# liuzm-slam/VLOAM-NOTED

Measured on AMD Instinct MI355X. Metric: scan-to-map LM iters/sec on 64-ring KITTI-shaped cloud, higher is better.
Workload: dtype fp64 pose/normal equations, fp32 points

## Files before the change

### vloam-noted_amd/csrc/mapper.hip

```cpp
#include <algorithm>
#include <cmath>
#include <cstdlib>
#include <array>
#include <cstring>
#include <deque>
#include <vector>

#include "common.h"
#include "device_math.h"
#include "cellhash.h"
#include "comm.h"
#include "cubeindex.h"
#include "lm.h"
#include "voxel.h"
#include "voxel_hot.h"
#include "voxel_pcl.h"
#include "mapper_dev.h"
#include "mapper_stack.h"
#include "mapper_frame.h"
#include "mapper_corr.h"
#include "mapper_lm.h"
#include "mapper_map.h"

namespace loam {
// ... 191 lines not shown
  while (p < v) p <<= 1;
  return p;
}

void free_all(loam_mapper* h) {
  if (h->D.lm_peer && h->comm) {
    comm_peer_release(h->comm);
    h->D.lm_peer = nullptr;
    h->D.lm_peer_flag = nullptr;
  }
  for (void* p : h->ipc_open) (void)hipIpcCloseMemHandle(p);
  h->ipc_open.clear();
  if (h->ipc_own) (void)hipFree(h->ipc_own);
  h->ipc_own = nullptr;
  h->D.ipc_tab = nullptr;
  for (void* p : h->allocs) (void)hipFree(p);
  h->allocs.clear();
  if (h->d_pub) (void)hipFree(h->d_pub);
  h->d_pub = nullptr;
  h->pub_cap = 0;
  for (auto& gp : h->gexec)
    for (auto& g : gp)
      if (g) (void)hipGraphExecDestroy(g);
  for (auto& e : h->ev_pool) (void)hipEventDestroy(e);
  if (h->ev_stack) (void)hipEventDestroy(h->ev_stack);
  for (ParitySlot& S : h->slot)
    for (hipEvent_t e : {S.ev_sin, S.ev_fr[0], S.ev_fr[1]})
      if (e) (void)hipEventDestroy(e);
  h->ev_pool.clear();
  if (h->ev_opt_begin) (void)hipEventDestroy(h->ev_opt_begin);
  if (h->ev_opt_end) (void)hipEventDestroy(h->ev_opt_end);
  if (h->st) (void)hipStreamDestroy(h->st);
  if (h->st2) (void)hipStreamDestroy(h->st2);
}

void host_initial_guess(HostStream& H, double* pose) {
  dq qm{H.q_wmap_wodom[0], H.q_wmap_wodom[1], H.q_wmap_wodom[2], H.q_wmap_wodom[3]};
  dq qo{H.q_wodom[0], H.q_wodom[1], H.q_wodom[2], H.q_wodom[3]};
  dq q = qmul(qm, qo);
  d3 r = qrot(qm, d3{H.t_wodom[0], H.t_wodom[1], H.t_wodom[2]});
  pose[0] = q.x; pose[1] = q.y; pose[2] = q.z; pose[3] = q.w;
  pose[4] = r.x + H.t_wmap_wodom[0];
  pose[5] = r.y + H.t_wmap_wodom[1];
  pose[6] = r.z + H.t_wmap_wodom[2];
}

void host_transform_update(HostStream& H) {
  dq qw{H.pose[0], H.pose[1], H.pose[2], H.pose[3]};
  dq qo{H.q_wodom[0], H.q_wodom[1], H.q_wodom[2], H.q_wodom[3]};
  dq qm = qmul(qw, qinv(qo));
  d3 r = qrot(qm, d3{H.t_wodom[0], H.t_wodom[1], H.t_wodom[2]});
  H.q_wmap_wodom[0] = qm.x; H.q_wmap_wodom[1] = qm.y; H.q_wmap_wodom[2] = qm.z; H.q_wmap_wodom[3] = qm.w;
  H.t_wmap_wodom[0] = H.pose[4] - r.x;
  H.t_wmap_wodom[1] = H.pose[5] - r.y;
  H.t_wmap_wodom[2] = H.pose[6] - r.z;
}

StreamFrame fresh_record() {
  StreamFrame F{};
  F.cen[0] = 10; F.cen[1] = 10; F.cen[2] = 5;
  F.pose[3] = F.wodom[3] = F.wmap[3] = 1.0;
  return F;
}

void pack7(const double* q, const double* t, double* x) {
  std::copy(q, q + 4, x);
  std::copy(t, t + 3, x + 4);
}
void unpack7(const double* x, double* q, double* t) {
  std::copy(x, x + 4, q);
  std::copy(x + 4, x + 7, t);
}

int32_t check_stream(loam_mapper* h, int32_t s) {
  if (!h) {
    set_error("null mapper handle");
    return LOAM_ERR_ARG;
  }
  if (s < 0 || s >= h->B) {
    set_error("stream index out of range");
    return LOAM_ERR_ARG;
  }
  return LOAM_OK;
}

void bind_stack_parity(const loam_mapper* h, MapperDev& D, int par) {
  const ParitySlot& S = h->slot[par];
  D.sin = S.sin_buf;
  D.stk_n = S.stk_n_buf;
  D.stk_err = S.stk_err_buf;
  for (int m = 0; m < 2; ++m) D.stack[m] = S.stack_buf[m];
}

}

extern "C" {

static int32_t ipc_peer_setup(loam_mapper* h) {
  loam_comm* c = h->comm;
  MapperDev& D = h->D;
  const int R = c->size, me = c->rank;
  const size_t B = h->B, nslot = 2 * B * 2 * LM_MAX_PASSES * LM_NACC;
  const size_t bytes = nslot * sizeof(double) + B * 2 * sizeof(uint32_t);
  struct Msg {
    hipIpcMemHandle_t hdl;
    int32_t ok, pad;
  };
  static_assert(sizeof(Msg) % 8 == 0, "exchange record");
  Msg mine{};
  void* buf = nullptr;
  if (hipExtMallocWithFlags(&buf, bytes, hipDeviceMallocUncached) != hipSuccess) {
    (void)hipGetLastError();
    buf = nullptr;
    if (hipMalloc(&buf, bytes) != hipSuccess) {
      (void)hipGetLastError();
      buf = nullptr;
    }
  }
  mine.ok = buf && hipMemset(buf, 0, bytes) == hipSuccess && hipDeviceSynchronize() == hipSuccess &&
            hipIpcGetMemHandle(&mine.hdl, buf) == hipSuccess;
  if (!mine.ok) (void)hipGetLastError();
  Msg* dsend = nullptr;
  Msg* drecv = nullptr;
  std::vector<Msg> all(R);
  auto cleanup = [&] {
    if (dsend) (void)hipFree(dsend);
    if (drecv) (void)hipFree(drecv);
    dsend = drecv = nullptr;
  };
  LOAM_HIP(hipMalloc(&dsend, sizeof(Msg)));
  if (hipMalloc(&drecv, sizeof(Msg) * R) != hipSuccess) {
    cleanup();
    return LOAM_ERR_HIP;
  }
  auto exchange = [&]() -> int32_t {
    if (hipMemcpy(dsend, &mine, sizeof(Msg), hipMemcpyHostToDevice) != hipSuccess) return LOAM_ERR_HIP;
    TRY(comm_allgather(c, dsend, drecv, (int64_t)sizeof(Msg), h->st));
    if (hipStreamSynchronize(h->st) != hipSuccess ||
        hipMemcpy(all.data(), drecv, sizeof(Msg) * R, hipMemcpyDeviceToHost) != hipSuccess)
      return LOAM_ERR_HIP;
    return LOAM_OK;
  };
  int32_t rc = exchange();
  bool ok = rc == LOAM_OK;
  for (int r = 0; r < R && ok; ++r) ok = all[r].ok != 0;
  std::vector<unsigned long long> tab(2 * (size_t)R, 0ull);
  if (ok) {
    for (int r = 0; r < R; ++r) {
      void* p = buf;
      if (r != me) {
        p = nullptr;
        if (hipIpcOpenMemHandle(&p, all[r].hdl, hipIpcMemLazyEnablePeerAccess) != hipSuccess) {
          (void)hipGetLastError();
          p = nullptr;
        } else {
          h->ipc_open.push_back(p);
        }
      }
      tab[r] = reinterpret_cast<unsigned long long>(p);
      tab[R + r] = p ? reinterpret_cast<unsigned long long>(static_cast<char*>(p) + nslot * sizeof(double)) : 0ull;
      if (!p) ok = false;
    }
    const hipIpcMemHandle_t keep = mine.hdl;
    mine = Msg{};
    mine.hdl = keep;
    mine.ok = ok ? 1 : 0;
    if (rc == LOAM_OK) rc = exchange();
    ok = rc == LOAM_OK;
    for (int r = 0; r < R && ok; ++r) ok = all[r].ok != 0;
  }
  cleanup();
  if (!ok) {
    for (void* p : h->ipc_open) (void)hipIpcCloseMemHandle(p);
    h->ipc_open.clear();
    if (buf) (void)hipFree(buf);
    return rc;
  }
  h->ipc_own = buf;
  unsigned long long* dtab = nullptr;
  const int32_t arc = dalloc(h, &dtab, tab.size());
  if (arc != LOAM_OK) return arc;
  LOAM_HIP(hipMemcpyAsync(dtab, tab.data(), sizeof(unsigned long long) * tab.size(), hipMemcpyHostToDevice, h->st));
  LOAM_HIP(hipStreamSynchronize(h->st));
  D.ipc_tab = dtab;
  D.ipc_B = (int)B;
  return LOAM_OK;
}

static int32_t mapper_create(const loam_params* p, int32_t device, int32_t n_streams, loam_comm* comm,
                             loam_mapper** out) {
  if (!out || n_streams <= 0) {
    set_error("loam_mapper_create: bad arguments");
    return LOAM_ERR_ARG;
  }
  *out = nullptr;
  TRY(ensure_device(device));
  LOAM_HIP(hipSetDevice(device));
  vh_spin_limit_from_env(device);
  lm_peer_spin_limit_from_env(device);
  auto* h = new loam_mapper;
  if (p) h->P = *p; else loam_params_default(&h->P);
  h->dev = device;
  h->B = n_streams;
  h->comm = comm;
  MapperDev& D = h->D;
  D.B = n_streams;
  if (comm) {
    D.sharded = 1;
    D.rank = comm->rank;
    D.nrank = comm->size;
  }
  D.max_in = h->P.max_input_points;
  D.map_cap = h->P.max_map_points;
  D.sub_cap = h->P.max_submap_points;
  D.scratch_cap = D.sub_cap + D.max_in;
  {
    const uint64_t cap = (uint64_t)D.map_cap, margin = (uint64_t)D.sub_cap + 2ull * D.max_in;
    h->compact_at = (uint32_t)std::max<uint64_t>(cap / 2, cap > margin ? cap - margin : 0);
    D.compact_at = h->compact_at;
    D.compact_due_at = h->compact_at;
  }
  D.max_chunks = LM_EBLK;
  {
    int occ = 0, cus = 0;
    const char* env = std::getenv("LOAM_LM_PERSISTENT");
    const bool allow = !(env && env[0] == '0');
    if (hipDeviceGetAttribute(&cus, hipDeviceAttributeMultiprocessorCount, device) == hipSuccess && cus > 0)
      h->n_cu = cus;
    const bool peer = comm && comm->size > 1 && comm->kind == 2;
    const char* ienv = std::getenv("LOAM_PEER_LM");
    const bool ipc = comm && comm->size > 1 && comm->kind != 2 && !(ienv && ienv[0] == '0');
    h->want_ipc = false;
    if (allow && (!comm || comm->size == 1 || peer || ipc) &&
        hipOccupancyMaxActiveBlocksPerMultiprocessor(&occ, k_lm_round, LM_THREADS, 0) == hipSuccess &&
        hipDeviceGetAttribute(&cus, hipDeviceAttributeMultiprocessorCount, device) == hipSuccess) {
      occ = std::min(occ, 1);
      const int cap = occ * cus;
      h->lm_G = std::min(LM_EBLK, std::min(16, cap / (peer ? lm_padded(n_streams) * comm->size : n_streams)));
      const char* genv = std::getenv("LOAM_LM_G");
      if (genv && std::atoi(genv) > 0) h->lm_G = std::min(LM_EBLK, std::atoi(genv));
      if (ipc && h->lm_G > 0) {
        if (lm_padded(n_streams) * comm->size <= cap) h->want_ipc = true;
        else h->lm_G = 0;
      }
      if (peer && h->lm_G > 0) {
        const size_t nd = (size_t)2 * n_streams * 2 * comm->size * LM_MAX_PASSES * LM_NACC;
        void* pb = nullptr;
        if (comm_peer_buffer(comm, nd * sizeof(double) + (size_t)n_streams * 2 * comm->size * sizeof(uint32_t),
                             lm_padded(n_streams) * comm->size, cap, &pb) == LOAM_OK) {
          D.lm_peer = static_cast<double*>(pb);
          D.lm_peer_flag = reinterpret_cast<uint32_t*>(D.lm_peer + nd);
        } else {
          h->lm_G = 0;
        }
      }
    }
  }
  D.pcl_order = h->P.exact_voxel_order ? 1 : 0;
  D.stack_k = (n_streams <= 4 && !D.pcl_order) ? 8 : 0;
  if (const char* kenv = std::getenv("LOAM_STACK_K"))
    if (D.stack_k) D.stack_k = std::max(1, std::min(STACK_K_MAX, std::atoi(kenv)));
  D.leaf[0] = (float)h->P.mapping_line_resolution;
  D.leaf[1] = (float)h->P.mapping_plane_resolution;
  const size_t B = n_streams;
  auto fail = [&](int32_t rc) {
    free_all(h);
    delete h;
    return rc;
  };
  int32_t rc = LOAM_OK;
#define ALLOC(ptr, n) \
  if ((rc = dalloc(h, &(ptr), (n))) != LOAM_OK) return fail(rc)
  if (hipStreamCreateWithFlags(&h->st, hipStreamNonBlocking) != hipSuccess) return fail(LOAM_ERR_HIP);
  if (hipStreamCreateWithFlags(&h->st2, hipStreamNonBlocking) != hipSuccess) return fail(LOAM_ERR_HIP);
  if (hipEventCreate(&h->ev_opt_begin) != hipSuccess || hipEventCreate(&h->ev_opt_end) != hipSuccess ||
      hipEventCreateWithFlags(&h->ev_stack, hipEventDisableTiming) != hipSuccess)
    return fail(LOAM_ERR_HIP);
  for (ParitySlot& S : h->slot)
    if (hipEventCreateWithFlags(&S.ev_sin, hipEventDisableTiming) != hipSuccess ||
        hipEventCreate(&S.ev_fr[0]) != hipSuccess || hipEventCreate(&S.ev_fr[1]) != hipSuccess)
      return fail(LOAM_ERR_HIP);
  {
    const char* denv = std::getenv("LOAM_DEFER_EVERY");
    D.defer_every = denv ? std::max(0, std::atoi(denv)) : 0;
  }
  h->use_graph = n_streams <= 4 ? 1 : 0;
  h->knn_cs = n_streams <= 4 ? 8 : 0;
  D.knn_blk = n_streams <= 4 ? 4 * CORR_BLK : CORR_BLK;
  if (const char* benv = std::getenv("LOAM_KNN_BLK"))
    if (h->knn_cs) D.knn_blk = std::max(1, std::min(64 * CORR_BLK, std::atoi(benv)));
  ALLOC(D.fr, B);
  for (int m = 0; m < 2; ++m) {
    ALLOC(D.in_pts[m], B * D.max_in);
    for (ParitySlot& S : h->slot) ALLOC(S.stack_buf[m], B * D.max_in);
  }
  ALLOC(D.arena, B * 2 * 2 * (size_t)D.map_cap);
  ALLOC(D.carena, B * 2 * 2 * (size_t)D.map_cap);
  ALLOC(D.ctab, B * 2 * 2 * 4 * (size_t)D.map_cap);
  ALLOC(h->cube_tab[0], B * 2 * NCUBE);
  ALLOC(h->cube_tab[1], B * 2 * NCUBE);
  ALLOC(D.extra_flag, B * 2 * NCUBE);
  D.knn_stride = B * 2 * (size_t)D.max_in;
  ALLOC(D.knn_id, 5 * D.knn_stride);
  ALLOC(D.r_type, B * 2 * (size_t)D.max_in);
  ALLOC(D.r_px, B * 2 * (size_t)D.max_in);
  ALLOC(D.r_py, B * 2 * (size_t)D.max_in);
  ALLOC(D.r_pz, B * 2 * (size_t)D.max_in);
  for (int k = 0; k < 3; ++k) {
    ALLOC(D.r_a[k], B * 2 * (size_t)D.max_in);
    ALLOC(D.r_b[k], B * 2 * (size_t)D.max_in);
  }
  ALLOC(D.ins_pts, B * 2 * (size_t)D.max_in);
  ALLOC(D.ins_tag, B * 2 * (size_t)D.max_in);
  ALLOC(D.ins_sorted, B * 2 * (size_t)D.max_in);
  ALLOC(D.ins_off, B * 2 * (size_t)(INS_SLOTS + 1));
  ALLOC(D.stable_tok, B * 2 * (size_t)NCUBE);
  ALLOC(h->tok_tmp, B * 2 * (size_t)NCUBE);
  ALLOC(D.dbg, LOAM_DEBUG_COUNTERS);
  {
    const char* penv = std::getenv("LOAM_PHASE_COUNTERS");
    D.pdbg = (penv && std::atoi(penv) > 0) ? D.dbg : nullptr;
  }
  ALLOC(D.vx_pts, B * 2 * (size_t)D.scratch_cap);
  if (D.pcl_order) {
    const size_t ps = mp_scratch(D);
    ALLOC(D.pe, B * 2 * ps);
    ALLOC(D.pa, B * 2 * ps);
    ALLOC(D.pb, B * 2 * ps);
    ALLOC(D.ps, B * 2 * ps);
    ALLOC(D.pseg, B * 2 * (mp_pseg(ps) + 9));
  }
  ALLOC(D.vx_idx, B * 2 * (size_t)D.scratch_cap);
  ALLOC(D.stk_part, B * 2 * (size_t)STACK_K_MAX);
  for (ParitySlot& S : h->slot) {
    ALLOC(S.stk_n_buf, B * 2);
    ALLOC(S.stk_err_buf, B);
    if (B <= 4) {
      if (!(S.sin_buf = S.hsin.assign_mapped(B, StackIn{}))) return fail(LOAM_ERR_HIP);
    } else {
      ALLOC(S.sin_buf, B);
      if (!S.hsin.assign(B, StackIn{})) return fail(LOAM_ERR_HIP);
    }
  }
  bind_stack_parity(h, D, 0);
  ALLOC(h->d_stk_ready, 2);
  ALLOC(D.stk_pts, B * 2 * (size_t)D.max_in);
  ALLOC(D.stk_idx, B * 2 * (size_t)D.max_in);
  ALLOC(D.partials, B * (size_t)D.max_chunks * LM_NACC);
  ALLOC(D.lm_sync, B * 2 * LM_SYNC_WORDS);
  ALLOC(D.lm_xpub, B * 2 * 8);
  ALLOC(D.tickets, B);
  ALLOC(D.lm_tick, B);
  D.rq_cap = B * 2 * INS_SLOTS;
  ALLOC(D.rq, (size_t)RQ_CLASSES * D.rq_cap);
  ALLOC(D.rq_ctl, RQ_CLASSES);
  ALLOC(h->d_map_off, 2 * NCUBE + 1);
  ALLOC(h->d_new_off, B * 2 * (NCUBE + 1));
  if (D.sharded) {
    for (int m = 0; m < 2; ++m) D.blk_v[m] = shard_block_voxels(D.leaf[m]);
    const size_t nq = B * 2 * (size_t)D.max_in;
    NnRec* recv = nullptr;
    ALLOC(D.wcnt, B * 2 * (size_t)WIN_MAX);
    ALLOC(D.nn_send, nq);
    if (D.nrank > 1) {
      ALLOC(recv, nq * D.nrank);
      D.nn_recv = recv;
    } else {
      D.nn_recv = D.nn_send;
    }
    ALLOC(D.nn_xyz, 5 * nq);
    ALLOC(D.lm_red, B * (size_t)LM_NACC);
    ALLOC(D.pose_x, (size_t)D.nrank * B * 8);
    ALLOC(h->d_q_off, B + 1);
    D.q_off = h->d_q_off;
    if (!h->q_off.assign(2 * (B + 1), 0)) return fail(LOAM_ERR_HIP);
    if (D.nrank == 1) {
      for (size_t s = 0; s <= B; ++s) h->q_off[s] = (int)(s * 2 * (size_t)D.max_in);
      if (hipMemcpyAsync(h->d_q_off, h->q_off.data(), sizeof(int) * (B + 1), hipMemcpyHostToDevice, h->st) !=
          hipSuccess)
        return fail(LOAM_ERR_HIP);
    }
  }
#undef ALLOC
  D.cube_tab = h->cube_tab[0];
  if (!h->hf.assign(B, StreamFrame{})) return fail(LOAM_ERR_HIP);
  for (ParitySlot& S : h->slot)
    if (!(S.hfo_dev = S.hfo.assign_mapped(B, StreamFrame{})) || !(S.fin_dev = S.fin.assign_mapped(B, FrameIn{})) ||
        !(S.hfo_early_dev = S.hfo_early.assign_mapped(B, StreamFrame{})))
      return fail(LOAM_ERR_HIP);
  if (!(h->done_dev = h->done.assign_mapped(2, 0ull)) || !(h->done_early_dev = h->done_early.assign_mapped(2, 0ull)))
    return fail(LOAM_ERR_HIP);
  h->hs.assign(B, HostStream{});
  h->last_tail.assign(B, std::array<uint32_t, 2>{0u, 0u});
  for (size_t s = 0; s < B; ++s) h->hf[s] = fresh_record();
  if (hipStreamSynchronize(h->st) != hipSuccess) return fail(LOAM_ERR_HIP);
  if (h->want_ipc) {
    if ((rc = ipc_peer_setup(h)) != LOAM_OK) return fail(rc);
    if (!D.ipc_tab) h->lm_G = 0;
  }
  *out = h;
  return LOAM_OK;
}

int32_t loam_mapper_create(const loam_params* p, int32_t device, int32_t n_streams, loam_mapper** out) {
  return mapper_create(p, device, n_streams, nullptr, out);
}

int32_t loam_mapper_create_sharded(const loam_params* p, int32_t device, int32_t n_streams, loam_comm* comm,
                                   loam_mapper** out) {
  if (!comm) {
    set_error("loam_mapper_create_sharded: null comm");
    return LOAM_ERR_ARG;
  }
  return mapper_create(p, device, n_streams, comm, out);
}

int32_t loam_shard_owner(const float* xyz, float leaf, int32_t nrank) {
  if (!xyz || !(leaf > 0.f) || nrank < 1) return LOAM_ERR_ARG;
  return shard_owner(xyz[0], xyz[1], xyz[2], 1.0f / leaf, shard_block_voxels(leaf), nrank);
}

static int32_t finish_oldest(loam_mapper* h);
static int32_t settle_all(loam_mapper* h);
static bool chain_capable(const loam_mapper* h);
#define SETTLE(h)                                \
  do {                                           \
    if ((h) && !(h)->q.empty()) {                \
      LOAM_HIP(hipSetDevice((h)->dev));          \
      TRY(settle_all(h));                        \
    }                                            \
  } while (0)
#define SETTLE_RESULTS(h)                                                                   \
  do {                                                                                      \
    if ((h) && !(h)->q.empty() && !(h)->q.front().behind && !(h)->q.front().early_seen) { \
      LOAM_HIP(hipSetDevice((h)->dev));                                                     \
      TRY(finish_oldest(h));                                                                \
    }                                                                                       \
  } while (0)

int32_t loam_mapper_destroy(loam_mapper* h) {
  if (!h) return LOAM_ERR_ARG;
  (void)hipSetDevice(h->dev);
  while (!h->q.empty()) (void)finish_oldest(h);
  (void)hipStreamSynchronize(h->st);
  (void)hipStreamSynchronize(h->st2);
  free_all(h);
  delete h;
  return LOAM_OK;
}

int32_t loam_mapper_reset(loam_mapper* h) {
  if (!h) return LOAM_ERR_ARG;
  SETTLE(h);
  LOAM_HIP(hipSetDevice(h->dev));
  LOAM_HIP(hipStreamSynchronize(h->st2));
  for (int p = 0; p < 2; ++p)
    LOAM_HIP(hipMemsetAsync(h->cube_tab[p], 0, sizeof(uint2) * h->B * 2 * NCUBE, h->st));
  LOAM_HIP(hipMemsetAsync(h->D.stable_tok, 0, sizeof(uint32_t) * h->B * 2 * NCUBE, h->st));
  LOAM_HIP(hipStreamSynchronize(h->st));
  for (int s = 0; s < h->B; ++s) {
    h->hf[s] = fresh_record();
    h->last_tail[s] = {0u, 0u};
    h->hs[s] = HostStream{};
  }
  return LOAM_OK;
}

static int32_t mapper_input_common(loam_mapper* h, int32_t s, const float* corner, int32_t nc,
                                   const float* surf, int32_t ns, const double* q_wodom,
                                   const double* t_wodom, int32_t skip, hipMemcpyKind kind) {
  TRY(check_stream(h, s));
  if (!q_wodom || !t_wodom || nc < 0 || ns < 0 || (nc > 0 && !corner) || (ns > 0 && !surf)) {
    set_error("loam_mapper_input: bad arguments");
    return LOAM_ERR_ARG;
  }
  if (nc > h->D.max_in || ns > h->D.max_in) {
    set_error("loam_mapper_input: cloud larger than max_input_points");
    return LOAM_ERR_CAPACITY;
  }
  LOAM_HIP(hipSetDevice(h->dev));
  HostStream& H = h->hs[s];
  if (skip) {
    SETTLE(h);
    for (int i = 0; i < 4; ++i) H.q_wodom[i] = q_wodom[i];
    for (int i = 0; i < 3; ++i) H.t_wodom[i] = t_wodom[i];
    H.skip = true;
    double pose[7];
    host_initial_guess(H, pose);
    unpack7(pose, H.q_hf, H.t_hf);
    H.in_ready = false;
    H.stk_launched = false;
    return LOAM_OK;
  }
  if (kind == hipMemcpyHostToDevice) {
    H.in_p[0] = h->D.in_pts[0] + (size_t)s * h->D.max_in;
    H.in_p[1] = h->D.in_pts[1] + (size_t)s * h->D.max_in;
    if (nc) LOAM_HIP(hipMemcpyAsync((void*)H.in_p[0], corner, sizeof(float4) * nc, kind, h->st2));
    if (ns) LOAM_HIP(hipMemcpyAsync((void*)H.in_p[1], surf, sizeof(float4) * ns, kind, h->st2));
  } else {
    H.in_p[0] = reinterpret_cast<const float4*>(corner);
    H.in_p[1] = reinterpret_cast<const float4*>(surf);
  }
  H.in_n[0] = nc;
  H.in_n[1] = ns;
  for (int i = 0; i < 4; ++i) H.in_q[i] = q_wodom[i];
  for (int i = 0; i < 3; ++i) H.in_t[i] = t_wodom[i];
  H.skip = false;
  H.in_ready = true;
  H.stk_launched = false;
  return LOAM_OK;
}

int32_t loam_mapper_input(loam_mapper* h, int32_t s, const float* corner, int32_t nc, const float* surf,
                          int32_t ns, const double* q_wodom, const double* t_wodom, int32_t skip) {
  return mapper_input_common(h, s, corner, nc, surf, ns, q_wodom, t_wodom, skip, hipMemcpyHostToDevice);
}

int32_t loam_mapper_input_device(loam_mapper* h, int32_t s, const float* corner, int32_t nc,
                                 const float* surf, int32_t ns, const double* q_wodom,
                                 const double* t_wodom, int32_t skip) {
  return mapper_input_common(h, s, corner, nc, surf, ns, q_wodom, t_wodom, skip, hipMemcpyDeviceToDevice);
}

static hipError_t prof_begin(loam_mapper* h, int fam, hipEvent_t* stop, hipStream_t st) {
  *stop = nullptr;
  if (!h->prof) return hipSuccess;
  size_t k = h->ev_fam.size() * 2;
  while (h->ev_pool.size() < k + 2) {
    hipEvent_t e;
    hipError_t err = hipEventCreate(&e);
    if (err != hipSuccess) return err;
    h->ev_pool.push_back(e);
  }
  h->ev_fam.push_back(fam);
  *stop = h->ev_pool[k + 1];
  return hipEventRecord(h->ev_pool[k], st);
}
struct ProfStop {
  hipEvent_t ev = nullptr;
  hipStream_t st = nullptr;
  hipError_t end() {
    const hipError_t e = ev ? hipEventRecord(ev, st) : hipSuccess;
    ev = nullptr;
    return e;
  }
  ~ProfStop() { (void)end(); }
};
#define LAUNCH_ON(stream, fam, ...)                     \
  do {                                                  \
    ProfStop stop_;                                     \
    stop_.st = (stream);                                \
    LOAM_HIP(prof_begin(h, (fam), &stop_.ev, (stream))); \
    __VA_ARGS__;                                        \
    LOAM_HIP(stop_.end());                              \
  } while (0)
#define LAUNCH(fam, ...) LAUNCH_ON(h->st, fam, __VA_ARGS__)

int32_t loam_mapper_input_device_batch(loam_mapper* h, int32_t n, const int32_t* streams,
                                       const uint64_t* d_corner, const int32_t* n_corner,
                                       const uint64_t* d_surf, const int32_t* n_surf,
                                       const double* q_wodom, const double* t_wodom) {
  if (!h || n < 0 || (n > 0 && (!streams || !d_corner || !n_corner || !d_surf || !n_surf || !q_wodom || !t_wodom))) {
    set_error("loam_mapper_input_device_batch: bad arguments");
    return LOAM_ERR_ARG;
  }
  for (int i = 0; i < n; ++i) {
    int32_t rc = mapper_input_common(h, streams[i], reinterpret_cast<const float*>(d_corner[i]), n_corner[i],
                                     reinterpret_cast<const float*>(d_surf[i]), n_surf[i], q_wodom + 4 * i,
                                     t_wodom + 3 * i, 0, hipMemcpyDeviceToDevice);
    if (rc != LOAM_OK) return rc;
  }
  return LOAM_OK;
}

int32_t loam_mapper_lm_path(loam_mapper* h) {
  if (!h) return LOAM_ERR_ARG;
  if (h->lm_G <= 0) return 0;
  if (h->D.lm_peer) return 2;
  if (h->D.ipc_tab) return 3;
  return 1;
}

int64_t loam_mapper_total_iterations(loam_mapper* h) {
  if (!h) return LOAM_ERR_ARG;
  SETTLE_RESULTS(h);
  int64_t it = 0;
  for (int s = 0; s < h->B; ++s)
    if (h->hs[s].solved_last) it += h->hs[s].st.lm[0].iterations + h->hs[s].st.lm[1].iterations;
  return it;
}

int32_t loam_mapper_stats_all(loam_mapper* h, loam_map_stats* out, int32_t n) {
  SETTLE_RESULTS(h);
  if (!h || !out || n < 0 || n > h->B) return LOAM_ERR_ARG;
  for (int s = 0; s < n; ++s) out[s] = h->hs[s].st;
  return LOAM_OK;
}

static int32_t launch_stacks(loam_mapper* h) {
  const int par = h->spar, B = h->B;
  for (const FrameRec& R : h->q)
    if (R.fpar == par) return LOAM_OK;
  bool any = false;
  ParitySlot& S = h->slot[par];
  LOAM_HIP(hipEventSynchronize(S.ev_sin));
  StackIn* in = S.hsin.data();
// ... 820 lines not shown
```

### vloam-noted_amd/csrc/mapper_corr.h

```cpp
#pragma once

namespace loam {

struct Near5 {
  float d[5];
  int id[5];
  int pos[5];
};
__device__ inline void near5_offer(Near5& T, float d, int id, int pos) {
  if (!(d < T.d[4] || (d == T.d[4] && id < T.id[4]))) return;
  T.d[4] = d; T.id[4] = id; T.pos[4] = pos;
#pragma unroll
  for (int k = 4; k > 0; --k) {
    if (T.d[k] < T.d[k - 1] || (T.d[k] == T.d[k - 1] && T.id[k] < T.id[k - 1])) {
      float td = T.d[k]; T.d[k] = T.d[k - 1]; T.d[k - 1] = td;
      int ti = T.id[k]; T.id[k] = T.id[k - 1]; T.id[k - 1] = ti;
      int tp = T.pos[k]; T.pos[k] = T.pos[k - 1]; T.pos[k - 1] = tp;
    }
  }
}
__device__ inline int floor_div50(int v) { return v >= 0 ? v / 50 : -((-v + 49) / 50); }

struct WinMap {
  uint32_t off[WIN_MAX], n[WIN_MAX], tsize[WIN_MAX];
  int sub[WIN_MAX];
};

__device__ inline void corr_block(const MapperDev& D, int* s, int* blk) {
  *s = D.s0 + blockIdx.x % D.B;
  *blk = blockIdx.x / D.B;
}

#ifndef KNN_WAVES
#define KNN_WAVES 7
#endif
template <int L, bool CS = false>
__global__ void __launch_bounds__(CORR_THREADS) __attribute__((amdgpu_waves_per_eu(CS ? 4 : KNN_WAVES, 8))) k_knn(MapperDev D, int round) {
  __shared__ WinMap W[2];
  __shared__ int slot_of[75];
  int s, blk;
  corr_block(D, &s, &blk);
  StreamFrame& F = D.fr[s];
  if (!F.active) return;
  double X[7];
#pragma unroll
  for (int i = 0; i < 7; ++i) X[i] = F.pose[i];
  if (blk == 0 && threadIdx.x < LM_SYNC_WORDS) D.lm_sync[((size_t)s * 2 + round) * LM_SYNC_WORDS + threadIdx.x] = 0;
  if (blk == 0 && threadIdx.x == 0) lm_init(F.lm[round], X, 4, F.optimize != 0);
  if (!F.optimize) return;
  const int tid = threadIdx.x;
  const int c0 = F.center[0] - 2, c1 = F.center[1] - 2, c2 = F.center[2] - 1;
  if (tid < 75) slot_of[tid] = -1;
  __syncthreads();
  if (tid < F.valid_num) {
    const int cube = F.window[tid];
    const int ci = cube % CW, cj = (cube / CW) % CH, ck = cube / (CW * CH);
    slot_of[(ci - c0) * 15 + (cj - c1) * 3 + (ck - c2)] = tid;
#pragma unroll
    for (int m = 0; m < 2; ++m) {
      const uint2 cv = D.cube_tab[sm_index(s, m) * NCUBE + cube];
      W[m].off[tid] = cv.x;
      W[m].n[tid] = cv.y;
      W[m].tsize[tid] = cv.y ? ci_table_size(cv.y) : 0u;
      W[m].sub[tid] = F.sub_off[m][tid];
    }
  }
  __syncthreads();
  const int nc = F.nc_stack, ns = F.ns_stack;
  const size_t rb = (size_t)s * 2 * D.max_in;
  uint32_t ncand = 0;
  const int gsub = tid % L;
  const int nblk = CS ? D.knn_blk : CORR_BLK;
  for (int ridx = blk * (CORR_THREADS / L) + tid / L; ridx < nc + ns; ridx += nblk * (CORR_THREADS / L)) {
    const int m = ridx < nc ? 0 : 1;
    const int qi = m == 0 ? ridx : ridx - nc;
    const float4 q = to_map(X, D.stack[m][(size_t)s * D.max_in + qi]);
    const float4* cp = carena_base(D, s, m, F.arena_active[m]);
    const uint2* ct = ctab_base(D, s, m, F.arena_active[m]);
    const WinMap& WM = W[m];
    Near5 T;
#pragma unroll
    for (int k = 0; k < 5; ++k) {
      T.d[k] = INFINITY;
      T.id[k] = 0x7FFFFFFF;
      T.pos[k] = -1;
    }
    const float fx = floorf(q.x), fy = floorf(q.y), fz = floorf(q.z);
    const int qx = (int)fx, qy = (int)fy, qz = (int)fz;
    const float lx = q.x - fx, hx = (fx + 1.0f) - q.x;
    const float ly = q.y - fy, hy = (fy + 1.0f) - q.y;
    const float lz = q.z - fz, hz = (fz + 1.0f) - q.z;
    auto scan = [&](int bi, int bj, int bk, int ax, int ay, int az) {
      const int wx = bi - c0, wy = bj - c1, wz = bk - c2;
      if (wx < 0 || wx > 4 || wy < 0 || wy > 4 || wz < 0 || wz > 2) return;
      const int sl = slot_of[wx * 15 + wy * 3 + wz];
      if (sl < 0) return;
      const uint32_t n = WM.n[sl];
      if (n == 0) return;
      const uint32_t off = WM.off[sl];
      const uint2 e = ci_find(ct + 4 * (size_t)off, WM.tsize[sl],
                              (uint32_t)ax | ((uint32_t)ay << 6) | ((uint32_t)az << 12));
      ncand += e.y;
      const int sub = WM.sub[sl];
      for (uint32_t k = CS ? 0 : gsub; k < e.y; k += CS ? 1 : L) {
        const uint32_t pos = off + e.x + k;
        const float4 p = cp[pos];
        const int key = (sub + __float_as_int(p.w)) * D.nrank + D.rank;
        near5_offer(T, fdist2(q.x, q.y, q.z, p.x, p.y, p.z), key, (int)pos);
      }
    };
    for (int ob = 0; ob < 27; ob += CS ? L : 1) {
      const int o = CS ? ob + gsub : ob;
      const uint32_t code = cell_order_code(o < 27 ? o : 0);
      const int dx = (int)(code & 3u) - 1, dy = (int)((code >> 2) & 3u) - 1, dz = (int)(code >> 4) - 1;
      const float gx = dx < 0 ? lx : (dx > 0 ? hx : 0.f);
      const float gy = dy < 0 ? ly : (dy > 0 ? hy : 0.f);
      const float gz = dz < 0 ? lz : (dz > 0 ? hz : 0.f);
      float bound = fminf(T.d[4], 1.0f) * 1.01f + 1e-6f;
#pragma unroll
      for (int o2 = 1; o2 < L; o2 <<= 1) bound = fminf(bound, __shfl_xor(bound, o2, 64));
      if (o >= 27 || gx * gx + gy * gy + gz * gz > bound) continue;
      const int x = qx + dx, y = qy + dy, z = qz + dz;
      const int bi = floor_div50(x + 25) + F.cen[0], bj = floor_div50(y + 25) + F.cen[1],
                bk = floor_div50(z + 25) + F.cen[2];
      int cx[3] = {bi, bj, bk};
      int lc[3];
      const int cv[3] = {x, y, z};
#pragma unroll
      for (int a = 0; a < 3; ++a) lc[a] = cv[a] - ci_corner(cx[a], F.cen[a]);
      scan(bi, bj, bk, lc[0], lc[1], lc[2]);
      int edge = 0;
#pragma unroll
      for (int a = 0; a < 3; ++a)
        if (cv[a] + 25 < 0 && (cv[a] + 25) % 50 == 0) edge |= 1 << a;
      for (int e = edge; e; e = (e - 1) & edge) {
        int b2[3], l2[3];
#pragma unroll
        for (int a = 0; a < 3; ++a) {
          b2[a] = (e >> a) & 1 ? cx[a] - 1 : cx[a];
          l2[a] = (e >> a) & 1 ? 50 : lc[a];
        }
        scan(b2[0], b2[1], b2[2], l2[0], l2[1], l2[2]);
      }
    }
#pragma unroll
    for (int o = 1; o < L; o <<= 1) {
      float pd[5];
      int pid[5], ppos[5];
#pragma unroll
      for (int k = 0; k < 5; ++k) {
        pd[k] = __shfl_xor(T.d[k], o, 64);
        pid[k] = __shfl_xor(T.id[k], o, 64);
        ppos[k] = __shfl_xor(T.pos[k], o, 64);
      }
#pragma unroll
      for (int k = 0; k < 5; ++k)
        if (ppos[k] >= 0) near5_offer(T, pd[k], pid[k], ppos[k]);
    }
    if (gsub != 0) continue;
    if (D.sharded) {
      NnRec& o = D.nn_send[D.q_off[s] + ridx];
#pragma unroll
      for (int k = 0; k < 5; ++k) {
        o.d[k] = T.d[k];
        o.id[k] = T.id[k];
        const float4 p = T.pos[k] >= 0 ? cp[T.pos[k]] : make_float4(0.f, 0.f, 0.f, 0.f);
        o.x[k] = p.x;
        o.y[k] = p.y;
        o.z[k] = p.z;
      }
      continue;
    }
    const bool ok = T.d[4] < 1.0f;
#pragma unroll
    for (int k = 0; k < 5; ++k) D.knn_id[k * D.knn_stride + rb + ridx] = ok ? T.pos[k] : -1;
  }
  unsigned long long wc = ncand;
#pragma unroll
  for (int o = 32; o > 0; o >>= 1) wc += __shfl_xor(wc, o, 64);
  if ((threadIdx.x & 63) == 0 && wc) atomicAdd(&F.cand[round], wc);
}

__global__ void __launch_bounds__(CORR_THREADS) k_nn_merge(MapperDev D) {
  const int s = D.s0 + blockIdx.x % D.B, blk = blockIdx.x / D.B;
  const StreamFrame& F = D.fr[s];
  if (!F.active || !F.optimize) return;
  const int nq = F.nc_stack + F.ns_stack;
  const size_t rb = (size_t)s * 2 * D.max_in;
  const size_t qtot = (size_t)D.q_off[D.s0 + D.B];
  for (int ridx = blk * CORR_THREADS + threadIdx.x; ridx < nq; ridx += CORR_BLK * CORR_THREADS) {
    Near5 T;
    float px[5], py[5], pz[5];
#pragma unroll
    for (int k = 0; k < 5; ++k) {
      T.d[k] = INFINITY;
      T.id[k] = 0x7FFFFFFF;
      T.pos[k] = -1;
      px[k] = py[k] = pz[k] = 0.f;
    }
    for (int r = 0; r < D.nrank; ++r) {
      const NnRec& c = D.nn_recv[(size_t)r * qtot + D.q_off[s] + ridx];
#pragma unroll
      for (int k = 0; k < 5; ++k) {
        const float d = c.d[k];
        const int id = c.id[k];
        if (!(d < T.d[4] || (d == T.d[4] && id < T.id[4]))) break;
        int j = 4;
        while (j > 0 && (d < T.d[j - 1] || (d == T.d[j - 1] && id < T.id[j - 1]))) {
          T.d[j] = T.d[j - 1];
          T.id[j] = T.id[j - 1];
          px[j] = px[j - 1];
          py[j] = py[j - 1];
          pz[j] = pz[j - 1];
          --j;
        }
        T.d[j] = d;
        T.id[j] = id;
        px[j] = c.x[k];
        py[j] = c.y[k];
        pz[j] = c.z[k];
      }
    }
    const bool ok = T.d[4] < 1.0f;
    D.knn_id[rb + ridx] = ok ? 0 : -1;
    if (ok) {
#pragma unroll
      for (int k = 0; k < 5; ++k) D.nn_xyz[k * D.knn_stride + rb + ridx] = make_float4(px[k], py[k], pz[k], 0.f);
    }
  }
}

__global__ void __launch_bounds__(CORR_THREADS) k_geom(MapperDev D, int round) {
  int s, blk;
  corr_block(D, &s, &blk);
  StreamFrame& F = D.fr[s];
  if (!F.active) return;
  const int nc = F.nc_stack, ns = F.ns_stack;
  const size_t rb = (size_t)s * 2 * D.max_in;
  uint32_t n_edge = 0, n_plane = 0;
  for (int ridx = blk * CORR_THREADS + threadIdx.x; ridx < nc + ns; ridx += CORR_BLK * CORR_THREADS) {
    if (!F.optimize) {
      D.r_type[rb + ridx] = 0;
      continue;
    }
    const int m = ridx < nc ? 0 : 1;
    const int qi = m == 0 ? ridx : ridx - nc;
    const float4 po = D.stack[m][(size_t)s * D.max_in + qi];
    int type = 0;
    double a[3] = {0, 0, 0}, b[3] = {0, 0, 0};
    if (D.knn_id[rb + ridx] >= 0) {
      const float4* lin = carena_base(D, s, m, F.arena_active[m]);
      float nb[5][3];
#pragma unroll
      for (int j = 0; j < 5; ++j) {
        const float4 p = D.sharded ? D.nn_xyz[j * D.knn_stride + rb + ridx] : lin[D.knn_id[j * D.knn_stride + rb + ridx]];
        nb[j][0] = p.x;
        nb[j][1] = p.y;
        nb[j][2] = p.z;
      }
      if (m == 0) {
        d3 pa, pb;
        if (edge_from_nbrs(nb, pa, pb)) {
          type = 1;
          d3 de{pa.x - pb.x, pa.y - pb.y, pa.z - pb.z};
          double dn = sqrt(de.x * de.x + de.y * de.y + de.z * de.z);
          a[0] = pa.x; a[1] = pa.y; a[2] = pa.z;
          b[0] = de.x / dn; b[1] = de.y / dn; b[2] = de.z / dn;
          ++n_edge;
        }
      } else {
        d3 n;
        double d;
        if (plane_from_nbrs(nb, n, d)) {
          type = 3;
          a[0] = n.x; a[1] = n.y; a[2] = n.z;
          b[0] = d;
          ++n_plane;
        }
      }
    }
    D.r_type[rb + ridx] = type;
    D.r_px[rb + ridx] = po.x;
    D.r_py[rb + ridx] = po.y;
    D.r_pz[rb + ridx] = po.z;
#pragma unroll
    for (int k = 0; k < 3; ++k) {
      D.r_a[k][rb + ridx] = a[k];
      D.r_b[k][rb + ridx] = b[k];
    }
  }
  uint32_t we = n_edge, wp = n_plane;
#pragma unroll
  for (int o = 32; o > 0; o >>= 1) {
    we += __shfl_xor(we, o, 64);
    wp += __shfl_xor(wp, o, 64);
  }
  if ((threadIdx.x & 63) == 0) {
    if (we) atomicAdd(&F.corner_num[round], (int)we);
    if (wp) atomicAdd(&F.surf_num[round], (int)wp);
  }
}

}
```

### vloam-noted_amd/csrc/mapper_dev.h

```cpp
#pragma once

namespace loam {

constexpr int CW = 21, CH = 21, CD = 11, NCUBE = CW * CH * CD;
constexpr int WIN_MAX = 125;
constexpr int WIN_VALID_MAX = 75;
constexpr int EXTRA_CAP = 64;
constexpr int CORR_THREADS = 128;
constexpr int CORR_BLK = 128;
static_assert(CORR_THREADS >= WIN_VALID_MAX, "k_knn window tables");
constexpr int LM_THREADS = 256;
constexpr int LM_EBLK = 32;
constexpr int INS_SLOTS = WIN_VALID_MAX + EXTRA_CAP;
constexpr int RQ_CLASSES = 8;
constexpr int MAP_ERR_SUBMAP = 4, MAP_ERR_EXTRA = 8, MAP_ERR_HASH = 16, MAP_ERR_LM_SYNC = 32,
              MAP_ERR_INDEX = 64, MAP_ERR_LIVE = 128, MAP_ERR_SORT = 256,
              MAP_ERR_STACK = 512, MAP_ERR_STACK_WAIT = 2048;

enum MapDbg {
  MD_REVOX_CYC = 0 , MD_MERGE_NEW_PTS = 3, MD_REVOX_ITEMS = 4 , MD_MERGES = 7,
  MD_INDEX_CYC = 8, MD_INDEX_PTS = 9, MD_OLD_PTS = 10, MD_CUBE_SEG = 11 , MD_INDEX_HASH_CYC = 16,
  MD_LM = 17 , MD_REVOX_SIZE_ITEMS = 24 , MD_REVOX_SIZE_CYC = 32 ,
  MD_POSE_DIFF = 40, MD_COMPACTIONS = 41, MD_STACK_SEG = 42 , MD_COMPACTIONS_MAP = 48 ,
  MD_CUBE_HOT = 50, MD_STACK_HOT = 54, MD_PREP_CYC = 58 ,
  MD_PREP_LAUNCHES = 62, MD_PREP_ON_DEVICE = 63, MD_CUBE_GLOB = 64, MD_STACK_GLOB = 65, MD_CUBE_HEAP = 66 ,
  MD_STACK_HEAP = 68 , MD_CUBE_SORT = 72, MD_STACK_SORT = 77, MD_CUBE_WAVES = 82, MD_STACK_CUTS = 91,
  MD_DBG_END = 92
};
static_assert(MD_POSE_DIFF == 40 && MD_COMPACTIONS == 41 && MD_COMPACTIONS_MAP + 1 == 49, "slots the tests read by number");
static_assert(MD_CUBE_HOT + VHF_SLOTS <= MD_STACK_HOT && MD_STACK_HOT + VHF_SLOTS <= MD_PREP_CYC &&
                  MD_CUBE_SORT + VHS_SLOTS == MD_STACK_SORT && MD_STACK_SORT + VHS_SLOTS == MD_CUBE_WAVES &&
                  MD_CUBE_WAVES + VHD_SLOTS == MD_STACK_CUTS && MD_CUBE_SEG + VXM_SLOTS <= MD_INDEX_HASH_CYC &&
                  MD_STACK_SEG + VXS_SLOTS == MD_COMPACTIONS_MAP && MD_DBG_END <= LOAM_DEBUG_COUNTERS,
              "counter slots");

struct StreamFrame {
  double pose[7];
  int active;
  uint32_t epoch;
  int nc_in, ns_in;
  int nc_stack, ns_stack;
  int sub_n[2];
  int optimize;
  int corner_num[2], surf_num[2];
  int valid_num;
  int window[WIN_MAX];
  int sub_off[2][WIN_MAX + 1];
  int center[3];
  int cen[3];
  int shift[3];
  int origin[3];
  uint32_t arena_tail[2];
  int arena_active[2];
  uint32_t scratch_tail[2];
  uint32_t hot_tail[2];
  int extra_n[2];
  int extra_list[2][EXTRA_CAP];
  int err;
  const float4* in_ptr[2];
  unsigned long long cand[2];
  unsigned long long vx_bytes;
  double wodom[7];
  double wmap[7];
  int deferred;
  LmState lm[2];
};

struct FrameIn {
  double wodom[7];
  const float4* in_ptr[2];
  int n[2];
  int active;
  int mode;
  uint32_t epoch;
  int pad;
  unsigned long long stack_seq;
};

struct StackIn {
  const float4* p[2];
  int n[2];
  int active;
  int pad;
};

struct MapPose {
  double x[7];
};

struct MapperDev {
  int B;
  int s0 = 0;
  int max_in, map_cap, sub_cap, scratch_cap, max_chunks;
  float leaf[2];
  uint32_t epoch;
  StreamFrame* fr;
  float4* in_pts[2];
  float4* stack[2];
  float4* arena;
  float4* carena;
  uint2* ctab;
  uint2* cube_tab;
  uint32_t* extra_flag;
  int* knn_id;
  size_t knn_stride;
  int* r_type;
  float* r_px;
  float* r_py;
  float* r_pz;
  double* r_a[3];
  double* r_b[3];
  float4* ins_pts;
  int* ins_tag;
  float4* ins_sorted;
  uint32_t* ins_off;
  unsigned long long* dbg;
  unsigned long long* pdbg;
  uint32_t* stable_tok;
  float4* vx_pts;
  int* vx_idx;
  double* partials;
  uint32_t* lm_sync;
  double* lm_xpub;
  uint32_t* tickets;
  uint32_t* lm_tick;
  uint32_t* rq;
  uint32_t* rq_ctl;
  int rq_cap = 0;
  uint32_t compact_at = 0;
  uint32_t compact_due_at = 0;
  int pcl_order = 0;
  uint64_t* pe;
  uint32_t* pa;
  uint32_t* pb;
  uint64_t* ps;
  int* pseg;
  int rank = 0, nrank = 1, sharded = 0;
  int blk_v[2] = {1, 1};
  uint32_t* wcnt;
  struct NnRec* nn_send;
  const struct NnRec* nn_recv;
  const int* q_off;
  float4* nn_xyz;
  double* pose_x;
  double* lm_red;
  double* lm_peer = nullptr;
  uint32_t* lm_peer_flag = nullptr;
  const unsigned long long* ipc_tab = nullptr;
  int ipc_B = 0;
  int stack_k = 0;
  uint2* stk_part;
  const StackIn* sin;
  int* stk_n;
  int* stk_err;
  float4* stk_pts;
  int* stk_idx;
  int knn_blk = CORR_BLK;
  const FrameIn* fin = nullptr;
  unsigned long long* stk_ready = nullptr;
  int defer_every = 0;
};

struct NnRec {
  float d[5];
  int id[5];
  float x[5], y[5], z[5];
};

__device__ inline size_t sm_index(int s, int m) { return (size_t)s * 2 + m; }

__device__ inline float4* arena_base(const MapperDev& D, int s, int m, int active) {
  return D.arena + ((sm_index(s, m) * 2 + active) * (size_t)D.map_cap);
}
__device__ inline float4* carena_base(const MapperDev& D, int s, int m, int active) {
  return D.carena + ((sm_index(s, m) * 2 + active) * (size_t)D.map_cap);
}
__device__ inline uint2* ctab_base(const MapperDev& D, int s, int m, int active) {
  return D.ctab + ((sm_index(s, m) * 2 + active) * (size_t)D.map_cap * 4);
}
__device__ inline void cube_corner(int c, const int* cen, int corner[3]) {
  corner[0] = ci_corner(c % CW, cen[0]);
  corner[1] = ci_corner((c / CW) % CH, cen[1]);
  corner[2] = ci_corner(c / (CW * CH), cen[2]);
}

__global__ void k_shift_cubes(MapperDev D, const uint2* __restrict__ old_tab, uint2* new_tab, uint32_t* tok_tmp) {
  int s = D.s0 + blockIdx.y;
  const StreamFrame& F = D.fr[s];
  for (int t = blockIdx.x * blockDim.x + threadIdx.x; t < 2 * NCUBE; t += gridDim.x * blockDim.x) {
    int m = t / NCUBE, c = t % NCUBE;
    int i = c % CW, j = (c / CW) % CH, k = c / (CW * CH);
    int oi = i - F.shift[0], oj = j - F.shift[1], ok = k - F.shift[2];
    uint2 v = make_uint2(0, 0);
    uint32_t tok = 0;
    if (oi >= 0 && oi < CW && oj >= 0 && oj < CH && ok >= 0 && ok < CD) {
      const size_t o = sm_index(s, m) * NCUBE + oi + CW * oj + CW * CH * ok;
      v = old_tab[o];
      tok = D.stable_tok[o];
    }
    new_tab[sm_index(s, m) * NCUBE + c] = v;
    tok_tmp[sm_index(s, m) * NCUBE + c] = tok;
  }
}

}
```

Measured before the change: 549,900.

## Reuse round-0 geometry in round 1 when KNN neighbor set is unchanged

In the second correspondence round, the KNN kernel compares the new five neighbor indices against the stored ones. It appends only the queries whose neighbors changed to a compacted redo list, using a wave ballot and one atomic per wave. k_geom then refits edge lines and plane normals only for that list and carries the round-0 corner/surface counts forward with corrections. This removes redundant eigen and plane fits for stable correspondences, at the cost of extra reads of old indices, atomics, and dependence on round-0 residuals still being valid, since the point positions are not re-transformed in this path.

Result: no change. 550,600 (median of 2 runs) (+0.1%).

```diff
diff --git a/vloam-noted_amd/csrc/mapper.hip b/vloam-noted_amd/csrc/mapper.hip
--- a/vloam-noted_amd/csrc/mapper.hip
+++ b/vloam-noted_amd/csrc/mapper.hip
@@ -517,6 +517,12 @@
   ALLOC(D.extra_flag, B * 2 * NCUBE);
   D.knn_stride = B * 2 * (size_t)D.max_in;
   ALLOC(D.knn_id, 5 * D.knn_stride);
+  ALLOC(D.knn_redo, D.knn_stride);
+  ALLOC(D.knn_redo_n, B);
+  {
+    const char* renv = std::getenv("LOAM_GEOM_REUSE");
+    D.geom_reuse = (!D.sharded && !(renv && renv[0] == '0')) ? 1 : 0;
+  }
   ALLOC(D.r_type, B * 2 * (size_t)D.max_in);
   ALLOC(D.r_px, B * 2 * (size_t)D.max_in);
   ALLOC(D.r_py, B * 2 * (size_t)D.max_in);
diff --git a/vloam-noted_amd/csrc/mapper_corr.h b/vloam-noted_amd/csrc/mapper_corr.h
--- a/vloam-noted_amd/csrc/mapper_corr.h
+++ b/vloam-noted_amd/csrc/mapper_corr.h
@@ -47,6 +47,7 @@
   for (int i = 0; i < 7; ++i) X[i] = F.pose[i];
   if (blk == 0 && threadIdx.x < LM_SYNC_WORDS) D.lm_sync[((size_t)s * 2 + round) * LM_SYNC_WORDS + threadIdx.x] = 0;
   if (blk == 0 && threadIdx.x == 0) lm_init(F.lm[round], X, 4, F.optimize != 0);
+  if (blk == 0 && threadIdx.x == 0 && round == 0) D.knn_redo_n[s] = 0;
   if (!F.optimize) return;
   const int tid = threadIdx.x;
   const int c0 = F.center[0] - 2, c1 = F.center[1] - 2, c2 = F.center[2] - 1;
@@ -172,8 +173,23 @@
       continue;
     }
     const bool ok = T.d[4] < 1.0f;
-#pragma unroll
-    for (int k = 0; k < 5; ++k) D.knn_id[k * D.knn_stride + rb + ridx] = ok ? T.pos[k] : -1;
+    int nid[5];
+#pragma unroll
+    for (int k = 0; k < 5; ++k) nid[k] = ok ? T.pos[k] : -1;
+    if (round == 1 && D.geom_reuse) {
+      int diff = 0;
+#pragma unroll
+      for (int k = 0; k < 5; ++k) diff |= D.knn_id[k * D.knn_stride + rb + ridx] ^ nid[k];
+      if (diff == 0) continue;
+      const unsigned long long changed = __ballot(1);
+      const int lane = threadIdx.x & 63, lead = __ffsll(changed) - 1;
+      uint32_t at = 0;
+      if (lane == lead) at = atomicAdd(&D.knn_redo_n[s], (uint32_t)__popcll(changed));
+      at = __shfl(at, lead, 64) + __popcll(changed & ((1ull << lane) - 1));
+      D.knn_redo[rb + at] = ridx;
+    }
+#pragma unroll
+    for (int k = 0; k < 5; ++k) D.knn_id[k * D.knn_stride + rb + ridx] = nid[k];
   }
   unsigned long long wc = ncand;
 #pragma unroll
@@ -237,11 +253,26 @@
   if (!F.active) return;
   const int nc = F.nc_stack, ns = F.ns_stack;
   const size_t rb = (size_t)s * 2 * D.max_in;
-  uint32_t n_edge = 0, n_plane = 0;
-  for (int ridx = blk * CORR_THREADS + threadIdx.x; ridx < nc + ns; ridx += CORR_BLK * CORR_THREADS) {
+  int n_edge = 0, n_plane = 0;
+  const bool reuse = round == 1 && D.geom_reuse;
+  if (reuse && !F.optimize) return;
+  const int nq = reuse ? (int)D.knn_redo_n[s] : nc + ns;
+  if (reuse && blk == 0 && threadIdx.x == 0) {
+    if (F.corner_num[0]) atomicAdd(&F.corner_num[1], F.corner_num[0]);
+    if (F.surf_num[0]) atomicAdd(&F.surf_num[1], F.surf_num[0]);
+    atomicAdd(&D.dbg[MD_GEOM_REUSED], (unsigned long long)(nc + ns - nq));
+    atomicAdd(&D.dbg[MD_GEOM_RECOMPUTED], (unsigned long long)nq);
+  }
+  for (int i = blk * CORR_THREADS + threadIdx.x; i < nq; i += CORR_BLK * CORR_THREADS) {
+    const int ridx = reuse ? D.knn_redo[rb + i] : i;
     if (!F.optimize) {
       D.r_type[rb + ridx] = 0;
       continue;
+    }
+    if (reuse) {
+      const int was = D.r_type[rb + ridx];
+      n_edge -= was == 1;
+      n_plane -= was == 3;
     }
     const int m = ridx < nc ? 0 : 1;
     const int qi = m == 0 ? ridx : ridx - nc;
@@ -289,16 +320,16 @@
       D.r_b[k][rb + ridx] = b[k];
     }
   }
-  uint32_t we = n_edge, wp = n_plane;
+  int we = n_edge, wp = n_plane;
 #pragma unroll
   for (int o = 32; o > 0; o >>= 1) {
     we += __shfl_xor(we, o, 64);
     wp += __shfl_xor(wp, o, 64);
   }
   if ((threadIdx.x & 63) == 0) {
-    if (we) atomicAdd(&F.corner_num[round], (int)we);
-    if (wp) atomicAdd(&F.surf_num[round], (int)wp);
-  }
-}
-
-}
+    if (we) atomicAdd(&F.corner_num[round], we);
+    if (wp) atomicAdd(&F.surf_num[round], wp);
+  }
+}
+
+}
diff --git a/vloam-noted_amd/csrc/mapper_dev.h b/vloam-noted_amd/csrc/mapper_dev.h
--- a/vloam-noted_amd/csrc/mapper_dev.h
+++ b/vloam-noted_amd/csrc/mapper_dev.h
@@ -25,7 +25,8 @@
   MD_CUBE_HOT = 50, MD_STACK_HOT = 54, MD_PREP_CYC = 58 ,
   MD_PREP_LAUNCHES = 62, MD_PREP_ON_DEVICE = 63, MD_CUBE_GLOB = 64, MD_STACK_GLOB = 65, MD_CUBE_HEAP = 66 ,
   MD_STACK_HEAP = 68 , MD_CUBE_SORT = 72, MD_STACK_SORT = 77, MD_CUBE_WAVES = 82, MD_STACK_CUTS = 91,
-  MD_DBG_END = 92
+  MD_GEOM_REUSED = 92, MD_GEOM_RECOMPUTED = 93 ,
+  MD_DBG_END = 94
 };
 static_assert(MD_POSE_DIFF == 40 && MD_COMPACTIONS == 41 && MD_COMPACTIONS_MAP + 1 == 49, "slots the tests read by number");
 static_assert(MD_CUBE_HOT + VHF_SLOTS <= MD_STACK_HOT && MD_STACK_HOT + VHF_SLOTS <= MD_PREP_CYC &&
@@ -104,6 +105,9 @@
   uint32_t* extra_flag;
   int* knn_id;
   size_t knn_stride;
+  int* knn_redo;
+  uint32_t* knn_redo_n;
+  int geom_reuse = 0;
   int* r_type;
   float* r_px;
   float* r_py;
```
